# smallflyingpig/speech-to-image-translation-without-text

Measured on AMD Instinct MI355X. Metric: StackGAN-v2 3-stage G+D train-step images/sec at 256px, higher is better.
Workload: dtype f32

## Files before the change

### include/s2i_hip.h

```cpp
#ifndef S2I_HIP_H
#define S2I_HIP_H

#include <stddef.h>
#include <stdint.h>

#ifdef __cplusplus
extern "C" {
#endif

#define S2I_ABI_VERSION 4

#define S2I_CONV_K1      0
#define S2I_CONV_K3S1    1
#define S2I_CONV_K4S2    2
#define S2I_TCONV_K4S2   3

#define S2I_CONV_1D      4

#define S2I_ACT_NONE     0
#define S2I_ACT_GLU      1
#define S2I_ACT_LRELU    2
#define S2I_ACT_TANH     3
#define S2I_ACT_RELU     4

// ... 37 lines not shown
                     void* stream);

int s2i_conv_forward_cls(const s2i_conv_desc* d, const float* x, const float* cvec, const float* w,
                         const float* bias, const float* cls_bias, float* y, float* part, void* ws,
                         size_t ws_bytes, void* stream);

int s2i_conv_forward_in(const s2i_conv_desc* d, const float* x_raw, const float* in_coef, const float* w, float* y,
                        float* part, void* ws, size_t ws_bytes, void* stream);

int s2i_cvec_bias_table(const float* cvec, const float* packed, int B, int Cc, int Ip, int Op, int N,
                        float* table, void* ws , size_t ws_bytes, void* stream);
size_t s2i_border_sums_workspace_bytes(int B, int H, int W, int C);
int s2i_tap_sums(const float* dy, int B, int H, int W, int C, float* tapsum, void* ws, size_t ws_bytes,
                 void* stream);
int s2i_cvec_grads(const float* cvec, const float* packed, const float* tapsum, int B, int Cc, int Ip,
                   int Op, int N, int O, int I_total, float* dc, float* dw_oihw, int accumulate,
                   void* stream);

typedef struct s2i_wgrad_desc {
  int kind;
  int B, H, W;
  int Ca;
  int Cc;
  int N;
  int ldg;
  int swap;
  int fold;
  int O, I, KH, KW;
  int accumulate;
  int i_off;
  int I_total;
  int a_act;
  int a_groups;
} s2i_wgrad_desc;

size_t s2i_wgrad_workspace_bytes(const s2i_wgrad_desc* d);
int s2i_conv_wgrad(const s2i_wgrad_desc* d, const float* a, const float* cvec, const float* g,
                   float* grad_oihw, void* ws, size_t ws_bytes, void* stream);

int s2i_conv_wgrad_in_eligible(const s2i_wgrad_desc* d);
int s2i_conv_wgrad_in(const s2i_wgrad_desc* d, const float* a_raw, const float* a_coef, const float* g,
                      float* grad_oihw, void* ws, size_t ws_bytes, void* stream);


int s2i_conv_split_eligible(const s2i_conv_desc* d);
int s2i_conv_forward_split(const s2i_conv_desc* d, const float* x, const float* cvec,
                           const unsigned short* wsplit, int planes, int np, int kp, const float* bias,
                           const float* cls_bias, float* y, float* part, void* ws, size_t ws_bytes,
                           void* stream);
size_t s2i_wgrad_workspace_bytes_split(const s2i_wgrad_desc* d, int planes);
int s2i_conv_wgrad_split(const s2i_wgrad_desc* d, int planes, const float* a, const float* cvec,
                         const float* g, float* grad_oihw, void* ws, size_t ws_bytes, void* stream);
int s2i_split_packed_weight(const float* packed, int T, int R, int C, int planes, unsigned short* out_rc,
                            unsigned short* out_cr, void* stream);


int    s2i_conv_bf16_eligible(const s2i_conv_desc* d);
size_t s2i_conv_bf16_workspace_bytes(const s2i_conv_desc* d);
int    s2i_conv_bf16_stat_parts(const s2i_conv_desc* d);
size_t s2i_conv_bf16_weight_elems(const s2i_conv_desc* d);
int    s2i_conv_bf16_weight_layout(const s2i_conv_desc* d);
int s2i_pack_conv_weight_bf16(const s2i_conv_desc* d, const float* packed, int R, int C, unsigned short* out,
                              void* stream);
typedef struct s2i_pack16_item {
  const float* P;
  unsigned short* out;
// ... 123 lines not shown
```

### speech_to_image_translation_without_text_amd/_lib.py

```python
import ctypes
import os

import torch

_HERE = os.path.dirname(os.path.abspath(__file__))
LIB_PATH = os.path.join(_HERE, "libs2i_hip.so")

CONV_K1, CONV_K3S1, CONV_K4S2, TCONV_K4S2, CONV_1D = 0, 1, 2, 3, 4
ACT_NONE, ACT_GLU, ACT_LRELU, ACT_TANH, ACT_RELU = 0, 1, 2, 3, 4
PACK_PLAIN, PACK_UPFOLD = 0, 1
DT_F32, DT_BF16 = 0, 1
ABI_VERSION = 4

c_int, c_float, c_void_p, c_size_t, c_ll = (ctypes.c_int, ctypes.c_float, ctypes.c_void_p,
                                            ctypes.c_size_t, ctypes.c_longlong)


class ConvDesc(ctypes.Structure):
    _fields_ = [(n, c_int) for n in ("kind", "B", "H", "W", "Cx", "Cc", "N", "wmode", "flip", "wR",
                                     "ldw", "act", "stats", "ldy", "groups", "nosplit", "kw", "stride", "pad",
                                     "tile_rows", "in_act", "in_groups")]


class WgradDesc(ctypes.Structure):
    _fields_ = [(n, c_int) for n in ("kind", "B", "H", "W", "Ca", "Cc", "N", "ldg", "swap", "fold",
                                     "O", "I", "KH", "KW", "accumulate", "i_off", "I_total", "a_act", "a_groups")]


class PackItem(ctypes.Structure):
    _fields_ = [("w", c_void_p), ("packed", c_void_p)] + [(n, c_int) for n in ("O", "I", "KH", "KW", "Ip", "mode", "gx",
                                                                               "block0")]


class Pack16Item(ctypes.Structure):
    _fields_ = [("P", c_void_p), ("out", c_void_p)] + [(n, c_int) for n in (
        "R", "C", "kind", "flip", "transpose", "T", "nphase", "Nn", "Npad", "Kk", "CK", "gx", "gy", "block0")]


P = c_void_p
_SIGNATURES = {
    "s2i_last_error": (ctypes.c_char_p, []),
    "s2i_version": (c_int, []),
    "s2i_check_device": (c_int, []),
    "s2i_set_tuning": (c_int, [ctypes.c_char_p, c_int]),
    "s2i_get_tuning": (c_int, [ctypes.c_char_p, ctypes.POINTER(c_int)]),
    "s2i_conv_workspace_bytes": (c_size_t, [ctypes.POINTER(ConvDesc)]),
    "s2i_conv_stat_parts": (c_int, [ctypes.POINTER(ConvDesc)]),
    "s2i_conv_forward": (c_int, [ctypes.POINTER(ConvDesc), P, P, P, P, P, P, P, c_size_t, P]),
    "s2i_conv_forward_cls": (c_int, [ctypes.POINTER(ConvDesc), P, P, P, P, P, P, P, P, c_size_t, P]),
    "s2i_conv_forward_in": (c_int, [ctypes.POINTER(ConvDesc), P, P, P, P, P, P, c_size_t, P]),
    "s2i_conv_wgrad_in_eligible": (c_int, [ctypes.POINTER(WgradDesc)]),
    "s2i_conv_wgrad_in": (c_int, [ctypes.POINTER(WgradDesc), P, P, P, P, P, c_size_t, P]),
    "s2i_conv_split_eligible": (c_int, [ctypes.POINTER(ConvDesc)]),
    "s2i_conv_forward_split": (c_int, [ctypes.POINTER(ConvDesc), P, P, P, c_int, c_int, c_int, P, P, P, P, P, c_size_t, P]),
    "s2i_split_packed_weight": (c_int, [P, c_int, c_int, c_int, c_int, P, P, P]),
    "s2i_wgrad_workspace_bytes_split": (c_size_t, [ctypes.POINTER(WgradDesc), c_int]),
    "s2i_conv_wgrad_split": (c_int, [ctypes.POINTER(WgradDesc), c_int, P, P, P, P, P, c_size_t, P]),
    "s2i_conv_bf16_eligible": (c_int, [ctypes.POINTER(ConvDesc)]),
    "s2i_conv_bf16_workspace_bytes": (c_size_t, [ctypes.POINTER(ConvDesc)]),
# ... 153 lines not shown
```

### speech_to_image_translation_without_text_amd/csrc/s2i_igemm.hip

```cpp
#include "s2i_common.h"

namespace {

struct IgemmP {
  const float* __restrict__ x;
  const float* __restrict__ cvec;
  const float* __restrict__ w;
  const float* __restrict__ bias;
  const float* __restrict__ cls_bias;
  float* __restrict__ y;
  float* __restrict__ part;
  float* __restrict__ slab;
  int B, H, W, Cx, Cc, Ca;
  int Ho, Wo, lgWo, lgHoWo;
  int M, N, K, T;
  int kind, flip, act, stats, splitk, cps, nchunks;
  int ldw, wR, ldy, nparts;
  int g_kw, g_s, g_pad;
  int wt;
  int x16, y16;
  unsigned x_bytes, c_bytes, w_bytes;
  long long Mrows;
  const unsigned short* __restrict__ wsp;
  int wsp_np, wsp_kp, wsp_plane;
// ... 1259 lines not shown
      } else {
        *reinterpret_cast<f32x4*>(y + row * ldy + quad * 4) = v;
      }
      s0 += v;
      s1 += v * v;
    }
  }
  sh[0][tid] = s0;
  sh[1][tid] = s1;
  __syncthreads();
  if (rl == 0 && quad < Q) {
    for (int r = 1; r < rpb; ++r) {
      s0 += sh[0][r * cpb + ql];
      s1 += sh[1][r * cpb + ql];
    }
    *reinterpret_cast<f32x4*>(part + ((size_t)0 * nparts + blockIdx.x) * N + quad * 4) = s0;
    *reinterpret_cast<f32x4*>(part + ((size_t)1 * nparts + blockIdx.x) * N + quad * 4) = s1;
  }
}

struct WgradP {
  const float* __restrict__ a;
  const float* __restrict__ cvec;
  const float* __restrict__ g;
  float* __restrict__ slab;
  int B, H, W, Ca, Cc, Cin;
  int Ho, Wo, lgWo, lgHoWo;
  int M, N, ldg, K, T, kind;
  int cps, nchunks;
  int a16, g16;
  unsigned a_bytes, c_bytes, g_bytes;
  const float* __restrict__ a_coef;
  int a_groups, a_ipg;
};

__device__ __forceinline__ void wgrad_block_map(int& tile, int& split) {
  const int tiles = gridDim.x * gridDim.y, nsplit = gridDim.z;
  const int L = blockIdx.x + gridDim.x * (blockIdx.y + gridDim.y * blockIdx.z);
  const int per_group = 8 * tiles;
  const int grp = L / per_group, Ll = L - grp * per_group;
  const int in_group = min(8, nsplit - grp * 8);
  split = grp * 8 + Ll % in_group;
  tile = Ll / in_group;
}

template <int BM, int BN, int WAVES_M, int WAVES_N, bool AACT = false>
__global__ __launch_bounds__(64 * WAVES_M * WAVES_N, (WAVES_M * WAVES_N > 4 ? 4 : 3)) void igemm_wgrad_kernel(WgradP p) {
  constexpr int TM = BM / (WAVES_M * 32), TN = BN / (WAVES_N * 32);
  constexpr int LDA = BM, LDB = BN;
  constexpr int NT = 64 * WAVES_M * WAVES_N;
  constexpr int AROWS = NT * 4 / BM, BROWS = NT * 4 / BN;
  static_assert(AROWS * BM == NT * 4 && BROWS * BN == NT * 4, "a pass must cover whole rows");
  constexpr int APASS = (32 + AROWS - 1) / AROWS, BPASS = (32 + BROWS - 1) / BROWS;
  constexpr bool APRED = (32 % AROWS) != 0, BPRED = (32 % BROWS) != 0;
  __shared__ __attribute__((aligned(16))) float smem[32 * LDA + 32 * LDB];
  float* As = smem;
  float* Bs = smem + 32 * LDA;
  const int tid = threadIdx.x, lane = tid & 63, wave = tid >> 6;
  const int wm = wave / WAVES_N, wn = wave % WAVES_N;
  int tile_, split;
  wgrad_block_map(tile_, split);
  const int k0 = (tile_ % gridDim.x) * BM, n0 = (tile_ / gridDim.x) * BN;
  int s, pad, kw;
  geom(p.kind, s, pad, kw);

  const int acol4 = tid % (BM / 4), arow = tid / (BM / 4);
  const int bcol4 = tid % (BN / 4), brow = tid / (BN / 4);
  const int kcol = k0 + acol4 * 4;
  const bool kvalid = kcol < p.K;
  int c = 0, dy = 0, dx = 0;
  if (kvalid) {
    const int t = kcol / p.Cin;
    c = kcol - t * p.Cin;
    dy = t / kw;
    dx = t - dy * kw;
  }
  const bool from_vec = c < p.Cc;
  const int nb = n0 + bcol4 * 4;
  const bool nvalid = nb < p.N;

  const __amdgpu_buffer_rsrc_t ra_rs = __builtin_amdgcn_make_buffer_rsrc((void*)p.a, 0, p.a_bytes, 0x00020000);
  const __amdgpu_buffer_rsrc_t rc_rs = __builtin_amdgcn_make_buffer_rsrc((void*)p.cvec, 0, p.c_bytes, 0x00020000);
  const __amdgpu_buffer_rsrc_t rg_rs = __builtin_amdgcn_make_buffer_rsrc((void*)p.g, 0, p.g_bytes, 0x00020000);
  const int acolb = (c - p.Cc) * 4;
  const int ccolb = c * 4;
  const int gcolb = nvalid ? nb * 4 : S2I_OOB;
  f32x4 ra[APASS], rb[BPASS];
  f32x4 gs[3], gt[3];
  unsigned apass = 0;
  if constexpr (AACT) {
#pragma unroll
    for (int g = 0; g < 3; ++g) {
      const int gg = g < p.a_groups ? g : 0;
      gs[g] = kvalid ? *reinterpret_cast<const f32x4*>(p.a_coef + ((size_t)gg * 4 + 2) * p.Ca + c) : f32x4{0.f, 0.f, 0.f, 0.f};
      gt[g] = kvalid ? *reinterpret_cast<const f32x4*>(p.a_coef + ((size_t)gg * 4 + 3) * p.Ca + c) : f32x4{0.f, 0.f, 0.f, 0.f};
    }
  }
  auto fetch = [&](int pc) {
    if constexpr (AACT) apass = 0;
#pragma unroll
    for (int q = 0; q < APASS; ++q) {
      const int m = pc * 32 + arow + q * AROWS;
      if (APRED && arow + q * AROWS >= 32) continue;
      const int b = m >> p.lgHoWo;
      const int r = m & ((1 << p.lgHoWo) - 1);
      const int oy = r >> p.lgWo, ox = r & (p.Wo - 1);
// ... 24 lines not shown

  const int c_begin = split * p.cps;
  const int c_end = min(p.nchunks, c_begin + p.cps);
  if (c_begin < c_end) fetch(c_begin);
  for (int pc = c_begin; pc < c_end; ++pc) {
#pragma unroll
    for (int q = 0; q < APASS; ++q)
      if (!APRED || arow + q * AROWS < 32) {
        f32x4 v = ra[q];
        if constexpr (AACT) {
          const unsigned bits = (apass >> (3 * q)) & 7u;
          const unsigned grp = bits & 3u;
          const f32x4 sc = grp == 0 ? gs[0] : (grp == 1 ? gs[1] : gs[2]);
          const f32x4 sh = grp == 0 ? gt[0] : (grp == 1 ? gt[1] : gt[2]);
#pragma unroll
          for (int j = 0; j < 4; ++j) {
            float z = fmaf(v[j], sc[j], sh[j]);
            z = z > 0.f ? z : 0.2f * z;
            v[j] = (bits & 4u) ? z : 0.f;
          }
        }
        *reinterpret_cast<f32x4*>(As + (arow + q * AROWS) * LDA + acol4 * 4) = v;
      }
#pragma unroll
    for (int q = 0; q < BPASS; ++q)
      if (!BPRED || brow + q * BROWS < 32) *reinterpret_cast<f32x4*>(Bs + (brow + q * BROWS) * LDB + bcol4 * 4) = rb[q];
    __syncthreads();
    if (pc + 1 < c_end) fetch(pc + 1);
    mma_chunk<TM, TN, LDA, LDB>(As, Bs, wm * TM * 32, wn * TN * 32, lane, acc);
    __syncthreads();
  }

  const int l31 = lane & 31, lh = lane >> 5;
  float* outp = p.slab + (size_t)split * p.K * p.N;
#pragma unroll
  for (int i = 0; i < TM; ++i)
#pragma unroll
    for (int r = 0; r < 16; ++r) {
      const int krow = k0 + wm * TM * 32 + i * 32 + (r & 3) + 8 * (r >> 2) + 4 * lh;
      if (krow >= p.K) continue;
#pragma unroll
      for (int j = 0; j < TN; ++j) {
        const int n = n0 + wn * TN * 32 + j * 32 + l31;
        if (n < p.N) outp[(size_t)krow * p.N + n] = acc[i][j][r];
      }
    }
}

typedef short s16x4 __attribute__((ext_vector_type(4)));
typedef short s16x8 __attribute__((ext_vector_type(8)));

__device__ __forceinline__ s16x4 lds_tr_read(const unsigned char* ptr) {
  return __builtin_amdgcn_ds_read_tr16_b64_v4i16((s16x4 __attribute__((address_space(3)))*)(ptr));
}

template <int BM, int BN, int WAVES_M, int WAVES_N, int NP>
__global__ __launch_bounds__(256, 3) void igemm_wgrad_split_kernel(WgradP p) {
  constexpr int TM = BM / (WAVES_M * 32), TN = BN / (WAVES_N * 32);
  constexpr int AROWB = BM * 2, BROWB = BN * 2;
  constexpr int APLANE = 32 * AROWB, BPLANE = 32 * BROWB;
  constexpr int AMASK = BM / 8 - 1, BMASK = BN / 8 - 1;
  constexpr int APASS = BM / 32, BPASS = BN / 32;
  constexpr int AROWS = 1024 / BM, BROWS = 1024 / BN;
  __shared__ __attribute__((aligned(16))) unsigned char smem[NP * (APLANE + BPLANE)];
  unsigned char* As = smem;
  unsigned char* Bs = smem + NP * APLANE;
// ... 477 lines not shown
    f32x4 g0[9], g1[9];
    const f32x4 av0 = load_a(m0), av1 = load_a(m1);
    load_g(m0, g0);
    load_g(m1, g1);
    fma9(av0, g0);
    fma9(av1, g1);
  }
  if (grp < ngroups) {
    const int m0 = grp * PPW + pl;
    f32x4 g0[9];
    const f32x4 av0 = load_a(m0);
    load_g(m0, g0);
    fma9(av0, g0);
  }
#pragma unroll
  for (int t = 0; t < 9; ++t)
#pragma unroll
    for (int j = 0; j < 4; ++j) {
      f32x4 v = acc[t][j];
#pragma unroll
      for (int sft = LPP; sft < 64; sft <<= 1)
#pragma unroll
        for (int n = 0; n < 4; ++n) v[n] += __shfl_xor(v[n], sft);
      if (pl == 0) red[wave][(t * LPP + q) * 4 + j] = v;
    }
  __syncthreads();
  float* outp = p.slab + (size_t)blockIdx.x * p.K * 4;
  for (int e = tid; e < 9 * LPP * 4; e += 256) {
    const f32x4 v = red[0][e] + red[1][e] + red[2][e] + red[3][e];
    *reinterpret_cast<f32x4*>(outp + (size_t)e * 4) = v;
  }
}

__global__ __launch_bounds__(256) void slab_sum_tree_kernel(float* __restrict__ slab, int S, int n4) {
  __shared__ f32x4 sh[256];
  const int tid = threadIdx.x;
  const int e = blockIdx.x * 4 + (tid & 3), sl = tid >> 2;
  f32x4 v = {0.f, 0.f, 0.f, 0.f};
  if (e < n4)
    for (int s = sl; s < S; s += 64) v += *reinterpret_cast<const f32x4*>(slab + ((size_t)s * n4 + e) * 4);
  sh[tid] = v;
  __syncthreads();
  for (int h = 32; h >= 1; h >>= 1) {
    if (sl < h) sh[tid] += sh[tid + h * 4];
    __syncthreads();
  }
  if (sl == 0 && e < n4) *reinterpret_cast<f32x4*>(slab + (size_t)e * 4) = sh[tid];
}

__global__ __launch_bounds__(256) void slab_sum_kernel(float* __restrict__ slab, int S, long long n4) {
  for (long long e = (long long)blockIdx.x * blockDim.x + threadIdx.x; e < n4;
       e += (long long)gridDim.x * blockDim.x) {
    f32x4 v = *reinterpret_cast<const f32x4*>(slab + e * 4);
    for (int s = 1; s < S; ++s) v += *reinterpret_cast<const f32x4*>(slab + ((size_t)s * n4 + e) * 4);
    *reinterpret_cast<f32x4*>(slab + e * 4) = v;
  }
}

__global__ __launch_bounds__(256) void wgrad_finish_kernel(const float* __restrict__ slab, int S, int K, int N,
                                                           int Cg, int O, int I, int Tp, int T, int swap, int fold,
                                                           int accumulate, int RT, float* __restrict__ grad,
                                                           int i_off, int I_total) {
  extern __shared__ float tile[];
  const int tid = threadIdx.x;
  const int ncols = swap ? I : O, nrows = swap ? O : I;
  const int c0 = blockIdx.x * 32, r0 = blockIdx.y * RT;
  const size_t sstride = (size_t)K * N;
  const int nload = T * RT * 32;
  for (int e = tid; e < nload; e += 256) {
    const int c_l = e & 31;
    const int r_l = (e >> 5) % RT;
    const int t = (e >> 5) / RT;
    const int c = c0 + c_l, r = r0 + r_l;
    float v = 0.f;
    if (c < ncols && r < nrows) {
      const float* sp = slab + ((size_t)t * Cg + r) * N + c;
      for (int s = 0; s < S; ++s) v += sp[s * sstride];
    }
    tile[(t * RT + r_l) * 33 + c_l] = v;
  }
  __syncthreads();
  const int nout = 32 * RT * Tp;
  for (int w = tid; w < nout; w += 256) {
    const int tapo = w % Tp;
    const int rest = w / Tp;
    int o_l, i_l, r_l, c_l;
    if (swap) { i_l = rest & 31; o_l = rest >> 5; r_l = o_l; c_l = i_l; }
    else { i_l = rest % RT; o_l = rest / RT; r_l = i_l; c_l = o_l; }
// ... 718 lines not shown
}

extern "C" size_t s2i_wgrad_workspace_bytes_dt(const s2i_wgrad_desc* d, int a_dtype, int g_dtype) {
  WgPlan pl;
  if (plan_wgrad(d, &pl, (a_dtype && g_dtype) ? 16 : ((a_dtype || g_dtype) ? 1 : 0))) return 0;
  return (size_t)pl.splitk * pl.K * d->N * sizeof(float);
}

extern "C" int s2i_conv_wgrad_dt(const s2i_wgrad_desc* d, const void* a, int a_dtype, const float* cvec, const void* g,
                                 int g_dtype, float* grad_oihw, void* ws, size_t ws_bytes, void* stream) {
  S2I_REQUIRE((a_dtype == S2I_DT_F32 || a_dtype == S2I_DT_BF16) && (g_dtype == S2I_DT_F32 || g_dtype == S2I_DT_BF16),
              "wgrad: unknown dtype");
  return conv_wgrad_impl(d, 0, (const float*)a, cvec, (const float*)g, grad_oihw, ws, ws_bytes, stream,
                         a_dtype == S2I_DT_BF16, g_dtype == S2I_DT_BF16);
}

extern "C" int s2i_conv_wgrad(const s2i_wgrad_desc* d, const float* a, const float* cvec, const float* g,
                              float* grad_oihw, void* ws, size_t ws_bytes, void* stream) {
  return conv_wgrad_impl(d, 0, a, cvec, g, grad_oihw, ws, ws_bytes, stream);
}

extern "C" size_t s2i_wgrad_workspace_bytes_split(const s2i_wgrad_desc* d, int planes) {
  WgPlan pl;
  if (plan_wgrad(d, &pl, planes)) return 0;
  return (size_t)pl.splitk * pl.K * d->N * sizeof(float);
}

extern "C" int s2i_conv_wgrad_split(const s2i_wgrad_desc* d, int planes, const float* a, const float* cvec,
                                    const float* g, float* grad_oihw, void* ws, size_t ws_bytes, void* stream) {
  S2I_REQUIRE(planes >= 1 && planes <= 3, "wgrad(split): need 1 to 3 bf16 planes");
  return conv_wgrad_impl(d, planes, a, cvec, g, grad_oihw, ws, ws_bytes, stream);
}

template <int BM, int BN, int WM, int WN>
static void launch_wgrad_split(const WgradP& p, dim3 grid, int planes, hipStream_t st) {
  if (planes == 1) hipLaunchKernelGGL((igemm_wgrad_split_kernel<BM, BN, WM, WN, 1>), grid, dim3(256), 0, st, p);
  else if (planes == 2) hipLaunchKernelGGL((igemm_wgrad_split_kernel<BM, BN, WM, WN, 2>), grid, dim3(256), 0, st, p);
  else hipLaunchKernelGGL((igemm_wgrad_split_kernel<BM, BN, WM, WN, 3>), grid, dim3(256), 0, st, p);
}

static int conv_wgrad_impl(const s2i_wgrad_desc* d, int planes, const float* a, const float* cvec, const float* g,
                           float* grad_oihw, void* ws, size_t ws_bytes, void* stream, int a16, int g16, const float* a_coef) {
  WgPlan pl;
  if (plan_wgrad(d, &pl, (a16 && g16) ? 16 : ((planes || a16 || g16) ? 1 : 0))) return 1;
  S2I_REQUIRE(!(planes && (a16 || g16)), "wgrad(split): bf16 tensors go through s2i_conv_wgrad_dt");
  S2I_REQUIRE(!(pl.small_n && g16), "wgrad: the <= 4 channel gradient stream expects an fp32 output gradient");
  S2I_REQUIRE((a || d->Ca == 0) && g && grad_oihw, "wgrad: null operand");
  S2I_REQUIRE(d->Cc == 0 || cvec != nullptr, "wgrad: cvec is null but Cc > 0");
  const size_t need = (size_t)pl.splitk * pl.K * d->N * sizeof(float);
  S2I_REQUIRE(ws && ws_bytes >= need, "wgrad: workspace too small (%zu < %zu)", ws_bytes, need);
  hipStream_t st = (hipStream_t)stream;
  WgradP p;
  p.a = a; p.cvec = cvec; p.g = g; p.slab = (float*)ws;
  p.B = d->B; p.H = d->H; p.W = d->W; p.Ca = d->Ca; p.Cc = d->Cc; p.Cin = pl.Cin;
  p.Ho = pl.Ho; p.Wo = pl.Wo; p.lgWo = s2i_ilog2(pl.Wo); p.lgHoWo = s2i_ilog2(pl.Ho * pl.Wo);
  p.M = pl.M; p.N = d->N; p.ldg = d->ldg; p.K = pl.K; p.T = pl.T; p.kind = d->kind;
  p.cps = pl.cps; p.nchunks = pl.nchunks;
  p.a16 = a16; p.g16 = g16;
  p.a_coef = a_coef; p.a_groups = d->a_groups < 1 ? 1 : d->a_groups; p.a_ipg = d->B / p.a_groups;
  if (a_coef) {
    S2I_REQUIRE(!planes && !a16 && !g16 && wgrad_in_ok(d, pl),
                "wgrad(apply-on-load): fp32 operands, LeakyReLU producer, no broadcast vector, 128 x 128 tile plan (check "
                "s2i_conv_wgrad_in_eligible)");
  }
  {
    const unsigned long long ab = (unsigned long long)d->B * d->H * d->W * d->Ca * (a16 ? 2ull : 4ull);
    const unsigned long long gb = (unsigned long long)pl.M * d->ldg * (g16 ? 2ull : 4ull);
    S2I_REQUIRE(ab < 0x7ff00000ull && gb < 0x7ff00000ull, "wgrad: tensor exceeds the 2 GiB buffer-addressing window");
    p.a_bytes = (unsigned)ab; p.g_bytes = (unsigned)gb;
    p.c_bytes = (unsigned)((unsigned long long)d->B * d->Cc * 4ull);
  }
  dim3 grid(pl.gridK, pl.gridN, pl.splitk);
  if (!a16 && g16 && d->kind == S2I_CONV_K4S2 && d->Ca == 4 && d->Cc == 0 && pl.K == 64 && d->N <= 64 && (d->N % 8) == 0 &&
      (d->ldg % 8) == 0) {
    WgradP q = p;
    q.nchunks = s2i_cdiv(pl.M, 64);
    q.cps = s2i_cdiv(q.nchunks, pl.splitk);
    dim3 g32(1, 1, s2i_cdiv(q.nchunks, q.cps));
    pl.splitk = (int)g32.z;
    pl.gridK = 1; pl.gridN = 1;
    hipLaunchKernelGGL((igemm_wgrad_b16_kernel<64, 64, 2, 2, true>), g32, dim3(256), 0, st, q);
  } else if (a16 && g16 && !pl.small_n && d->Cc == 0 && (pl.Cin % 8) == 0 && (d->N % 8) == 0 && (d->ldg % 8) == 0) {
    WgradP q = p;
    q.nchunks = s2i_cdiv(pl.M, 64);
    q.cps = s2i_cdiv(q.nchunks, pl.splitk);
    dim3 g16grid(pl.gridK, pl.gridN, s2i_cdiv(q.nchunks, q.cps));
    S2I_REQUIRE((int)g16grid.z <= pl.splitk, "wgrad(bf16): split plan mismatch");
    pl.splitk = (int)g16grid.z;
    if (pl.tile == 7) hipLaunchKernelGGL((igemm_wgrad_b16_kernel<256, 256, 4, 4>), g16grid, dim3(1024), 0, st, q);
    else if (pl.tile == 6) hipLaunchKernelGGL((igemm_wgrad_b16_kernel<256, 128, 4, 2>), g16grid, dim3(512), 0, st, q);
    else if (pl.tile == 0) hipLaunchKernelGGL((igemm_wgrad_b16_kernel<128, 128, 2, 2>), g16grid, dim3(256), 0, st, q);
    else if (pl.tile == 1) hipLaunchKernelGGL((igemm_wgrad_b16_kernel<128, 64, 2, 2>), g16grid, dim3(256), 0, st, q);
    else if (pl.tile == 2) hipLaunchKernelGGL((igemm_wgrad_b16_kernel<128, 32, 4, 1>), g16grid, dim3(256), 0, st, q);
    else hipLaunchKernelGGL((igemm_wgrad_b16_kernel<64, 64, 2, 2>), g16grid, dim3(256), 0, st, q);
  } else if (pl.rows3) {
    dim3 g3(d->Ca == 32 ? 1 : 3, pl.gridN, pl.splitk);
    if (d->Ca == 32 && pl.bn3 == 64) hipLaunchKernelGGL((wgrad_k3_rows_kernel<32, 64, 3, 1, 3>), g3, dim3(192), 0, st, p);
    else if (d->Ca == 32) hipLaunchKernelGGL((wgrad_k3_rows_kernel<32, 32, 3, 1, 3>), g3, dim3(192), 0, st, p);
    else if (pl.bn3 == 128) hipLaunchKernelGGL((wgrad_k3_rows_kernel<64, 128, 2, 2, 1>), g3, dim3(256), 0, st, p);
    else if (pl.bn3 == 64) hipLaunchKernelGGL((wgrad_k3_rows_kernel<64, 64, 2, 2, 1>), g3, dim3(256), 0, st, p);
    else hipLaunchKernelGGL((wgrad_k3_rows_kernel<64, 32, 2, 1, 1>), g3, dim3(128), 0, st, p);
  } else if (planes && !pl.small_n) {
    if (pl.tile == 0) launch_wgrad_split<128, 128, 2, 2>(p, grid, planes, st);
    else if (pl.tile == 1) launch_wgrad_split<128, 64, 2, 2>(p, grid, planes, st);
    else if (pl.tile == 2) launch_wgrad_split<128, 32, 4, 1>(p, grid, planes, st);
    else launch_wgrad_split<64, 64, 2, 2>(p, grid, planes, st);
  } else if (pl.small_n) {
    if (d->Ca == 16) hipLaunchKernelGGL(small_n_wgrad_kernel<4>, dim3(pl.splitk), dim3(256), 0, st, p);
    else if (d->Ca == 32) hipLaunchKernelGGL(small_n_wgrad_kernel<8>, dim3(pl.splitk), dim3(256), 0, st, p);
    else hipLaunchKernelGGL(small_n_wgrad_kernel<16>, dim3(pl.splitk), dim3(256), 0, st, p);
  } else if (pl.tile == 9) hipLaunchKernelGGL((igemm_wgrad_kernel<256, 256, 4, 4>), grid, dim3(1024), 0, st, p);
  else if (pl.tile == 8) hipLaunchKernelGGL((igemm_wgrad_kernel<256, 128, 4, 2>), grid, dim3(512), 0, st, p);
  else if (pl.tile == 0 && a_coef) hipLaunchKernelGGL((igemm_wgrad_kernel<128, 128, 2, 2, true>), grid, dim3(256), 0, st, p);
  else if (pl.tile == 0) hipLaunchKernelGGL((igemm_wgrad_kernel<128, 128, 2, 2>), grid, dim3(256), 0, st, p);
  else if (pl.tile == 1) hipLaunchKernelGGL((igemm_wgrad_kernel<128, 64, 2, 2>), grid, dim3(256), 0, st, p);
  else if (pl.tile == 2) hipLaunchKernelGGL((igemm_wgrad_kernel<128, 32, 4, 1>), grid, dim3(256), 0, st, p);
  else if (pl.tile == 3) hipLaunchKernelGGL((igemm_wgrad_kernel<64, 64, 2, 2>), grid, dim3(256), 0, st, p);
  else if (pl.tile == 4) hipLaunchKernelGGL((igemm_wgrad_kernel<96, 64, 3, 1>), grid, dim3(192), 0, st, p);
  else hipLaunchKernelGGL((igemm_wgrad_kernel<96, 32, 3, 1>), grid, dim3(192), 0, st, p);
  S2I_LAUNCH_CHECK("igemm_wgrad");
  {
    const int ncols = d->swap ? d->I : d->O, nrows = d->swap ? d->O : d->I;
    int RT = 8;
    while (RT > 1 && (long long)s2i_cdiv(ncols, 32) * s2i_cdiv(nrows, RT) < 128) RT >>= 1;
    dim3 fgrid(s2i_cdiv(ncols, 32), s2i_cdiv(nrows, RT));
    const size_t shb = (size_t)pl.T * RT * 33 * sizeof(float);
    int S = pl.splitk;
    const long long kn = (long long)pl.K * d->N;
    if (pl.small_n || (S >= 32 && (kn % 4) == 0 && kn / 4 < (1 << 18))) {
      hipLaunchKernelGGL(slab_sum_tree_kernel, dim3(s2i_cdiv(kn / 4, 4)), dim3(256), 0, st, (float*)ws, S, (int)(kn / 4));
      S2I_LAUNCH_CHECK("slab_sum_tree");
      S = 1;
    } else if (S > 2 && (kn % 4) == 0) {
      int sb = s2i_cdiv(kn / 4, 256);
      if (sb > 4096) sb = 4096;
      hipLaunchKernelGGL(slab_sum_kernel, dim3(sb), dim3(256), 0, st, (float*)ws, S, kn / 4);
      S2I_LAUNCH_CHECK("slab_sum");
      S = 1;
    }
    hipLaunchKernelGGL(wgrad_finish_kernel, fgrid, dim3(256), shb, st, (const float*)ws, S, pl.K, d->N,
                       pl.Cin, d->O, d->I, d->KH * d->KW, pl.T, d->swap, d->fold, d->accumulate, RT, grad_oihw,
                       d->i_off, d->I_total > 0 ? d->I_total : d->I);
  }
  S2I_LAUNCH_CHECK("wgrad_finish");
  return 0;
}

extern "C" int s2i_pack_conv_weights_batched(const s2i_pack_item* items_dev, int n, int total_blocks, int max_taps,
                                             void* stream) {
  S2I_REQUIRE(items_dev && n > 0 && total_blocks > 0 && max_taps > 0 && max_taps <= 16, "pack(batched): bad args");
  const size_t shb = (size_t)64 * (8 * max_taps + 1) * sizeof(float);
  hipLaunchKernelGGL(pack_weight_batched_kernel, dim3(total_blocks), dim3(256), shb, (hipStream_t)stream, items_dev, n);
  S2I_LAUNCH_CHECK("pack_weight_batched");
  return 0;
}

extern "C" int s2i_pack_conv_weight(const float* w_oihw, float* packed, int O, int I, int KH, int KW, int Ip,
                                    int mode, void* stream) {
  S2I_REQUIRE(w_oihw && packed, "pack: null pointer");
  S2I_REQUIRE(O > 0 && I > 0 && KH > 0 && KW > 0 && Ip >= I, "pack: bad shape");
  int T = KH * KW;
  if (mode == S2I_PACK_UPFOLD) {
    S2I_REQUIRE(KH == 3 && KW == 3, "pack: UPFOLD needs a 3x3 parameter");
    T = 16;
  } else {
    S2I_REQUIRE(mode == S2I_PACK_PLAIN, "pack: unknown mode %d", mode);
  }
  const int Op = (O + 3) & ~3;
  {
// ... 9 lines not shown
```

### speech_to_image_translation_without_text_amd/ops.py

```python
import ctypes
import os

import torch

from . import _lib
from ._lib import (ACT_GLU, ACT_LRELU, ACT_NONE, CONV_K1, CONV_K3S1, CONV_K4S2, DT_BF16, DT_F32,
                   PACK_PLAIN, PACK_UPFOLD, TCONV_K4S2, ConvDesc, WgradDesc, check, ptr, stream)

BN_EPS = 1e-5
BN_MOMENTUM = 0.1

DIRECT_PARAM_GRAD = False


def _direct(p):
    return (DIRECT_PARAM_GRAD and p is not None and p.requires_grad and p.grad is not None
            and p.grad.is_contiguous())


class param_grad_mode:

    def __init__(self, direct=True):
        self.new = bool(direct)

# ... 371 lines not shown
    y = torch.empty((B, Ho, Wo, N), dtype=torch.float32, device=x.device)
    if EXEC_LOG is not None:
        T = kw1 if conv1d is not None else _TAPS[kind]
        _log_exec("conv k%d %s[%d,%d,%d,%d+%d]->%d" % (kind, "T" if wmode else "", B, H, W, Cx, Cc, N), B * Ho * Wo, N,
                  T * (Cx + Cc), x.numel(), T * (Cx + Cc) * N * (4 if kind == TCONV_K4S2 else 1), y.numel())
    part, nparts = None, 0
    if stats:
        nparts = lib.s2i_conv_stat_parts(ctypes.byref(d))
        if nparts <= 0:
            check(1, "s2i_conv_stat_parts")
        part = torch.empty((2, nparts, N), dtype=torch.float32, device=x.device)
    wsb = lib.s2i_conv_workspace_bytes(ctypes.byref(d))
    ws = _ws.get(wsb, x.device)
    if (MATH_PLANES and in_src is None and w_offset == 0 and packed.dim() == 3
            and getattr(packed, '_s2i_gen', None) is not None and lib.s2i_conv_split_eligible(ctypes.byref(d))):
        transpose = wmode == 0
        np_, kp = (packed.shape[2], packed.shape[1]) if transpose else (packed.shape[1], packed.shape[2])
        if kp % 8 == 0:
            wsp = split_weight(packed, MATH_PLANES, transpose)
            check(lib.s2i_conv_forward_split(ctypes.byref(d), ptr(x), ptr(cvec), ptr(wsp), MATH_PLANES, np_, kp, ptr(bias),
                                             ptr(cls_bias), ptr(y), ptr(part), ptr(ws), ws.numel() * 4, stream()),
                  "s2i_conv_forward_split")
            return y, part, nparts
    wp = ptr(packed) + 4 * int(w_offset)
    if in_src is not None:
        check(lib.s2i_conv_forward_in(ctypes.byref(d), ptr(x), ptr(in_src.coef), wp, ptr(y), ptr(part), ptr(ws),
                                      ws.numel() * 4, stream()), "s2i_conv_forward_in")
        return y, part, nparts
    check(lib.s2i_conv_forward_cls(ctypes.byref(d), ptr(x), ptr(cvec), wp, ptr(bias), ptr(cls_bias), ptr(y), ptr(part),
                                   ptr(ws), ws.numel() * 4, stream()), "s2i_conv_forward")
    return y, part, nparts


def wgrad_raw(kind, a, cvec, g, grad_shape, *, swap=0, fold=0, out=None, accumulate=False, i_off=0, I_total=0, a_src=None):
    lib = _lib_ready()
    B, H, W, Ca = a.shape
    Cc = 0 if cvec is None else cvec.shape[1]
    N = g.shape[-1]
    if len(grad_shape) == 2:
        O, I, KH, KW = grad_shape[0], grad_shape[1], 1, 1
    else:
        O, I, KH, KW = grad_shape
    d = WgradDesc(kind, B, H, W, Ca, Cc, N, N, swap, fold, O, I, KH, KW, 1 if accumulate else 0, i_off, I_total,
                  a_src.act if a_src is not None else 0, a_src.groups if a_src is not None else 0)
    if EXEC_LOG is not None:
        Ho, Wo = _geom(kind, H, W)
        _log_exec("wgrad k%d a[%d,%d,%d,%d+%d] g%d" % (kind, B, H, W, Ca, Cc, N), B * Ho * Wo, N, _TAPS[kind] * (Ca + Cc),
                  a.numel(), g.numel(), _TAPS[kind] * (Ca + Cc) * N)
    if out is None:
        full = grad_shape if not I_total else (O, I_total, KH, KW)
        out = torch.empty(full, dtype=torch.float32, device=a.device)
    if a_src is not None:
        wsb = lib.s2i_wgrad_workspace_bytes(ctypes.byref(d))
        if wsb == 0:
            check(1, "s2i_wgrad_workspace_bytes")
        ws = _ws.get(wsb, a.device)
        check(lib.s2i_conv_wgrad_in(ctypes.byref(d), ptr(a), ptr(a_src.coef), ptr(g), ptr(out), ptr(ws), ws.numel() * 4,
                                    stream()), "s2i_conv_wgrad_in")
        return out
    if MATH_PLANES:
        wsb = lib.s2i_wgrad_workspace_bytes_split(ctypes.byref(d), MATH_PLANES)
        if wsb == 0:
            check(1, "s2i_wgrad_workspace_bytes_split")
        ws = _ws.get(wsb, a.device)
        check(lib.s2i_conv_wgrad_split(ctypes.byref(d), MATH_PLANES, ptr(a), ptr(cvec), ptr(g), ptr(out), ptr(ws),
                                       ws.numel() * 4, stream()), "s2i_conv_wgrad_split")
        return out
    wsb = lib.s2i_wgrad_workspace_bytes(ctypes.byref(d))
    if wsb == 0:
        check(1, "s2i_wgrad_workspace_bytes")
    ws = _ws.get(wsb, a.device)
    check(lib.s2i_conv_wgrad(ctypes.byref(d), ptr(a), ptr(cvec), ptr(g), ptr(out), ptr(ws), ws.numel() * 4,
                             stream()), "s2i_conv_wgrad")
    return out


def _rows_view(t):
# ... 617 lines not shown
```

Measured before the change: 748.4.

## Write conv wgrad results directly in OIHW layout, fusing the relayout and tap fold

```diff
diff --git a/include/s2i_hip.h b/include/s2i_hip.h
--- a/include/s2i_hip.h
+++ b/include/s2i_hip.h
@@ -93,6 +93,7 @@
   int I_total;
   int a_act;
   int a_groups;
+  int slab_finish;
 } s2i_wgrad_desc;
 
 size_t s2i_wgrad_workspace_bytes(const s2i_wgrad_desc* d);
diff --git a/speech_to_image_translation_without_text_amd/_lib.py b/speech_to_image_translation_without_text_amd/_lib.py
--- a/speech_to_image_translation_without_text_amd/_lib.py
+++ b/speech_to_image_translation_without_text_amd/_lib.py
@@ -24,7 +24,8 @@
 
 class WgradDesc(ctypes.Structure):
     _fields_ = [(n, c_int) for n in ("kind", "B", "H", "W", "Ca", "Cc", "N", "ldg", "swap", "fold",
-                                     "O", "I", "KH", "KW", "accumulate", "i_off", "I_total", "a_act", "a_groups")]
+                                     "O", "I", "KH", "KW", "accumulate", "i_off", "I_total", "a_act", "a_groups",
+                                     "slab_finish")]
 
 
 class PackItem(ctypes.Structure):
diff --git a/speech_to_image_translation_without_text_amd/csrc/s2i_igemm.hip b/speech_to_image_translation_without_text_amd/csrc/s2i_igemm.hip
--- a/speech_to_image_translation_without_text_amd/csrc/s2i_igemm.hip
+++ b/speech_to_image_translation_without_text_amd/csrc/s2i_igemm.hip
@@ -1315,6 +1315,9 @@
   unsigned a_bytes, c_bytes, g_bytes;
   const float* __restrict__ a_coef;
   int a_groups, a_ipg;
+  float* __restrict__ grad;
+  int I_total, i_off, accumulate;
+  int fold;
 };
 
 __device__ __forceinline__ void wgrad_block_map(int& tile, int& split) {
@@ -1327,7 +1330,7 @@
   tile = Ll / in_group;
 }
 
-template <int BM, int BN, int WAVES_M, int WAVES_N, bool AACT = false>
+template <int BM, int BN, int WAVES_M, int WAVES_N, bool AACT = false, bool OIHW = false>
 __global__ __launch_bounds__(64 * WAVES_M * WAVES_N, (WAVES_M * WAVES_N > 4 ? 4 : 3)) void igemm_wgrad_kernel(WgradP p) {
   constexpr int TM = BM / (WAVES_M * 32), TN = BN / (WAVES_N * 32);
   constexpr int LDA = BM, LDB = BN;
@@ -1352,9 +1355,17 @@
   const int kcol = k0 + acol4 * 4;
   const bool kvalid = kcol < p.K;
   int c = 0, dy = 0, dx = 0;
+  constexpr int OG = BM / 16;
   if (kvalid) {
-    const int t = kcol / p.Cin;
-    c = kcol - t * p.Cin;
+    int t;
+    if constexpr (OIHW) {
+      const int rl = acol4 * 4;
+      t = rl / OG;
+      c = k0 / 16 + rl % OG;
+    } else {
+      t = kcol / p.Cin;
+      c = kcol - t * p.Cin;
+    }
     dy = t / kw;
     dx = t - dy * kw;
   }
@@ -1445,6 +1456,58 @@
   }
 
   const int l31 = lane & 31, lh = lane >> 5;
+  if constexpr (OIHW) {
+    constexpr int LDT = BM + 4;
+    const bool one = gridDim.z == 1;
+    float* dst = one ? p.grad + (size_t)p.i_off * 16 : p.slab + (size_t)split * p.K * p.N;
+    const size_t ostride = one ? (size_t)p.I_total * 16 : (size_t)p.Cin * 16;
+    dst += k0;
+#pragma unroll
+    for (int cw = 0; cw < WAVES_N; ++cw)
+#pragma unroll
+      for (int j = 0; j < TN; ++j) {
+        __syncthreads();
+        if (wn == cw) {
+#pragma unroll
+          for (int i = 0; i < TM; ++i)
+#pragma unroll
+            for (int r = 0; r < 16; ++r) {
+              const int row = wm * TM * 32 + i * 32 + (r & 3) + 8 * (r >> 2) + 4 * lh;
+              smem[l31 * LDT + (row % OG) * 16 + row / OG] = acc[i][j][r];
+            }
+        }
+        __syncthreads();
+        for (int e = (one && p.fold) ? NT * 32 * BM : tid; e < 32 * (BM / 4); e += NT) {
+          const int col = e / (BM / 4), q = e - col * (BM / 4);
+          const int n = n0 + cw * TN * 32 + j * 32 + col;
+          if (n >= p.N) continue;
+          f32x4 v = *reinterpret_cast<const f32x4*>(smem + col * LDT + q * 4);
+          f32x4* gp = reinterpret_cast<f32x4*>(dst + (size_t)n * ostride + q * 4);
+          if (one) {
+            v = f32x4{0.f, 0.f, 0.f, 0.f} + v;
+            if (p.accumulate) v = *gp + v;
+          }
+          *gp = v;
+        }
+        if (one && p.fold) {
+          for (int e = tid; e < OG * 32 * 9; e += NT) {
+            const int ol = e / 288, rest = e - ol * 288, col = rest / 9, tap = rest - col * 9;
+            const int n = n0 + cw * TN * 32 + j * 32 + col;
+            if (n >= p.N) continue;
+            const float* x = smem + col * LDT + ol * 16;
+            const int ky = tap / 3, kx = tap - ky * 3;
+            float v = 0.f;
+#pragma unroll
+            for (int ay = 0; ay < 2; ++ay)
+#pragma unroll
+              for (int ax = 0; ax < 2; ++ax) v += 0.f + x[((2 - ky) + ay) * 4 + (2 - kx) + ax];
+            float* gp = p.grad + ((size_t)(k0 / 16 + ol) * p.I_total + p.i_off + n) * 9 + tap;
+            *gp = p.accumulate ? *gp + v : v;
+          }
+        }
+      }
+    return;
+  }
   float* outp = p.slab + (size_t)split * p.K * p.N;
 #pragma unroll
   for (int i = 0; i < TM; ++i)
@@ -1988,7 +2051,44 @@
   }
 }
 
-__global__ __launch_bounds__(256) void slab_sum_tree_kernel(float* __restrict__ slab, int S, int n4) {
+struct SlabToGrad {
+  float* grad;
+  int run, gstride, goff, accumulate;
+  int fold;
+};
+
+__device__ __forceinline__ void slab_fold_store(const SlabToGrad& og, long long grp, const f32x4 (&x)[4]) {
+  const long long i = grp / og.run, o = grp - i * og.run;
+  float* gp = og.grad + ((size_t)o * og.gstride + og.goff + i) * 9;
+#pragma unroll
+  for (int tap = 0; tap < 9; ++tap) {
+    const int ky = tap / 3, kx = tap - ky * 3;
+    float v = 0.f;
+#pragma unroll
+    for (int ay = 0; ay < 2; ++ay)
+#pragma unroll
+      for (int ax = 0; ax < 2; ++ax) {
+        const int t = ((2 - ky) + ay) * 4 + (2 - kx) + ax;
+        v += 0.f + x[t >> 2][t & 3];
+      }
+    gp[tap] = og.accumulate ? gp[tap] + v : v;
+  }
+}
+
+__device__ __forceinline__ void slab_sum_store(float* __restrict__ slab, const SlabToGrad& og, long long e4, f32x4 v) {
+  if (!og.grad) {
+    *reinterpret_cast<f32x4*>(slab + e4 * 4) = v;
+    return;
+  }
+  const long long e = e4 * 4;
+  const long long o = e / og.run;
+  f32x4* gp = reinterpret_cast<f32x4*>(og.grad + o * og.gstride + og.goff + (e - o * og.run));
+  v = f32x4{0.f, 0.f, 0.f, 0.f} + v;
+  if (og.accumulate) v = *gp + v;
+  *gp = v;
+}
+
+__global__ __launch_bounds__(256) void slab_sum_tree_kernel(float* __restrict__ slab, int S, int n4, SlabToGrad og) {
   __shared__ f32x4 sh[256];
   const int tid = threadIdx.x;
   const int e = blockIdx.x * 4 + (tid & 3), sl = tid >> 2;
@@ -2001,15 +2101,34 @@
     if (sl < h) sh[tid] += sh[tid + h * 4];
     __syncthreads();
   }
-  if (sl == 0 && e < n4) *reinterpret_cast<f32x4*>(slab + (size_t)e * 4) = sh[tid];
-}
-
-__global__ __launch_bounds__(256) void slab_sum_kernel(float* __restrict__ slab, int S, long long n4) {
+  if (og.fold) {
+    if (tid == 0 && e < n4) {
+      const f32x4 x[4] = {sh[0], sh[1], sh[2], sh[3]};
+      slab_fold_store(og, blockIdx.x, x);
+    }
+    return;
+  }
+  if (sl == 0 && e < n4) slab_sum_store(slab, og, e, sh[tid]);
+}
+
+__global__ __launch_bounds__(256) void slab_sum_kernel(float* __restrict__ slab, int S, long long n4, SlabToGrad og) {
+  if (og.fold) {
+    for (long long g = (long long)blockIdx.x * blockDim.x + threadIdx.x; g < n4 / 4; g += (long long)gridDim.x * blockDim.x) {
+      f32x4 x[4];
+#pragma unroll
+      for (int q = 0; q < 4; ++q) {
+        x[q] = *reinterpret_cast<const f32x4*>(slab + (g * 4 + q) * 4);
+        for (int s = 1; s < S; ++s) x[q] += *reinterpret_cast<const f32x4*>(slab + ((size_t)s * n4 + g * 4 + q) * 4);
+      }
+      slab_fold_store(og, g, x);
+    }
+    return;
+  }
   for (long long e = (long long)blockIdx.x * blockDim.x + threadIdx.x; e < n4;
        e += (long long)gridDim.x * blockDim.x) {
     f32x4 v = *reinterpret_cast<const f32x4*>(slab + e * 4);
     for (int s = 1; s < S; ++s) v += *reinterpret_cast<const f32x4*>(slab + ((size_t)s * n4 + e) * 4);
-    *reinterpret_cast<f32x4*>(slab + e * 4) = v;
+    slab_sum_store(slab, og, e, v);
   }
 }
 
@@ -2794,6 +2913,19 @@
   return conv_wgrad_impl(d, planes, a, cvec, g, grad_oihw, ws, ws_bytes, stream);
 }
 
+static bool wgrad_oihw_ok(const s2i_wgrad_desc* d, const WgPlan& pl, int planes, int a16, int g16) {
+  if (d->slab_finish || planes || a16 || g16 || pl.rows3 || pl.small_n) return false;
+  if (d->kind != S2I_CONV_K4S2 || d->Cc != 0) return false;
+  if (d->swap && d->fold) {
+    if (d->KH != 3 || d->KW != 3 || pl.Cin != d->O || d->N != d->I) return false;
+  } else if (d->swap || d->fold || d->KH != 4 || d->KW != 4 || pl.Cin != d->I || d->N != d->O) {
+    return false;
+  }
+  const int BM = pl.tile == 3 ? 64 : ((pl.tile == 8 || pl.tile == 9) ? 256 : 128);
+  if (!(pl.tile <= 3 || pl.tile == 8 || pl.tile == 9)) return false;
+  return (pl.K % BM) == 0;
+}
+
 template <int BM, int BN, int WM, int WN>
 static void launch_wgrad_split(const WgradP& p, dim3 grid, int planes, hipStream_t st) {
   if (planes == 1) hipLaunchKernelGGL((igemm_wgrad_split_kernel<BM, BN, WM, WN, 1>), grid, dim3(256), 0, st, p);
@@ -2820,6 +2952,9 @@
   p.cps = pl.cps; p.nchunks = pl.nchunks;
   p.a16 = a16; p.g16 = g16;
   p.a_coef = a_coef; p.a_groups = d->a_groups < 1 ? 1 : d->a_groups; p.a_ipg = d->B / p.a_groups;
+  p.grad = grad_oihw; p.I_total = d->I_total > 0 ? d->I_total : d->I; p.i_off = d->i_off; p.accumulate = d->accumulate;
+  p.fold = d->fold;
+  const bool oihw = wgrad_oihw_ok(d, pl, planes, a16, g16);
   if (a_coef) {
     S2I_REQUIRE(!planes && !a16 && !g16 && wgrad_in_ok(d, pl),
                 "wgrad(apply-on-load): fp32 operands, LeakyReLU producer, no broadcast vector, 128 x 128 tile plan (check "
@@ -2871,6 +3006,15 @@
     if (d->Ca == 16) hipLaunchKernelGGL(small_n_wgrad_kernel<4>, dim3(pl.splitk), dim3(256), 0, st, p);
     else if (d->Ca == 32) hipLaunchKernelGGL(small_n_wgrad_kernel<8>, dim3(pl.splitk), dim3(256), 0, st, p);
     else hipLaunchKernelGGL(small_n_wgrad_kernel<16>, dim3(pl.splitk), dim3(256), 0, st, p);
+  } else if (oihw) {
+    if (pl.tile == 9) hipLaunchKernelGGL((igemm_wgrad_kernel<256, 256, 4, 4, false, true>), grid, dim3(1024), 0, st, p);
+    else if (pl.tile == 8) hipLaunchKernelGGL((igemm_wgrad_kernel<256, 128, 4, 2, false, true>), grid, dim3(512), 0, st, p);
+    else if (pl.tile == 0 && a_coef)
+      hipLaunchKernelGGL((igemm_wgrad_kernel<128, 128, 2, 2, true, true>), grid, dim3(256), 0, st, p);
+    else if (pl.tile == 0) hipLaunchKernelGGL((igemm_wgrad_kernel<128, 128, 2, 2, false, true>), grid, dim3(256), 0, st, p);
+    else if (pl.tile == 1) hipLaunchKernelGGL((igemm_wgrad_kernel<128, 64, 2, 2, false, true>), grid, dim3(256), 0, st, p);
+    else if (pl.tile == 2) hipLaunchKernelGGL((igemm_wgrad_kernel<128, 32, 4, 1, false, true>), grid, dim3(256), 0, st, p);
+    else hipLaunchKernelGGL((igemm_wgrad_kernel<64, 64, 2, 2, false, true>), grid, dim3(256), 0, st, p);
   } else if (pl.tile == 9) hipLaunchKernelGGL((igemm_wgrad_kernel<256, 256, 4, 4>), grid, dim3(1024), 0, st, p);
   else if (pl.tile == 8) hipLaunchKernelGGL((igemm_wgrad_kernel<256, 128, 4, 2>), grid, dim3(512), 0, st, p);
   else if (pl.tile == 0 && a_coef) hipLaunchKernelGGL((igemm_wgrad_kernel<128, 128, 2, 2, true>), grid, dim3(256), 0, st, p);
@@ -2881,7 +3025,24 @@
   else if (pl.tile == 4) hipLaunchKernelGGL((igemm_wgrad_kernel<96, 64, 3, 1>), grid, dim3(192), 0, st, p);
   else hipLaunchKernelGGL((igemm_wgrad_kernel<96, 32, 3, 1>), grid, dim3(192), 0, st, p);
   S2I_LAUNCH_CHECK("igemm_wgrad");
+  if (oihw) {
+    const int S = pl.splitk;
+    const long long kn = (long long)pl.K * d->N;
+    const SlabToGrad og = d->fold ? SlabToGrad{grad_oihw, pl.Cin, p.I_total, d->i_off, d->accumulate, 1}
+                                  : SlabToGrad{grad_oihw, pl.K, p.I_total * 16, d->i_off * 16, d->accumulate, 0};
+    if (S >= 32 && kn / 4 < (1 << 18)) {
+      hipLaunchKernelGGL(slab_sum_tree_kernel, dim3(s2i_cdiv(kn / 4, 4)), dim3(256), 0, st, (float*)ws, S, (int)(kn / 4), og);
+      S2I_LAUNCH_CHECK("slab_sum_tree");
+    } else if (S > 1) {
+      int sb = s2i_cdiv(d->fold ? kn / 16 : kn / 4, 256);
+      if (sb > 4096) sb = 4096;
+      hipLaunchKernelGGL(slab_sum_kernel, dim3(sb), dim3(256), 0, st, (float*)ws, S, kn / 4, og);
+      S2I_LAUNCH_CHECK("slab_sum");
+    }
+    return 0;
+  }
   {
+    const SlabToGrad to_slab{nullptr, 1, 0, 0, 0, 0};
     const int ncols = d->swap ? d->I : d->O, nrows = d->swap ? d->O : d->I;
     int RT = 8;
     while (RT > 1 && (long long)s2i_cdiv(ncols, 32) * s2i_cdiv(nrows, RT) < 128) RT >>= 1;
@@ -2890,13 +3051,13 @@
     int S = pl.splitk;
     const long long kn = (long long)pl.K * d->N;
     if (pl.small_n || (S >= 32 && (kn % 4) == 0 && kn / 4 < (1 << 18))) {
-      hipLaunchKernelGGL(slab_sum_tree_kernel, dim3(s2i_cdiv(kn / 4, 4)), dim3(256), 0, st, (float*)ws, S, (int)(kn / 4));
+      hipLaunchKernelGGL(slab_sum_tree_kernel, dim3(s2i_cdiv(kn / 4, 4)), dim3(256), 0, st, (float*)ws, S, (int)(kn / 4), to_slab);
       S2I_LAUNCH_CHECK("slab_sum_tree");
       S = 1;
     } else if (S > 2 && (kn % 4) == 0) {
       int sb = s2i_cdiv(kn / 4, 256);
       if (sb > 4096) sb = 4096;
-      hipLaunchKernelGGL(slab_sum_kernel, dim3(sb), dim3(256), 0, st, (float*)ws, S, kn / 4);
+      hipLaunchKernelGGL(slab_sum_kernel, dim3(sb), dim3(256), 0, st, (float*)ws, S, kn / 4, to_slab);
       S2I_LAUNCH_CHECK("slab_sum");
       S = 1;
     }
diff --git a/speech_to_image_translation_without_text_amd/ops.py b/speech_to_image_translation_without_text_amd/ops.py
--- a/speech_to_image_translation_without_text_amd/ops.py
+++ b/speech_to_image_translation_without_text_amd/ops.py
@@ -427,7 +427,8 @@
     return y, part, nparts
 
 
-def wgrad_raw(kind, a, cvec, g, grad_shape, *, swap=0, fold=0, out=None, accumulate=False, i_off=0, I_total=0, a_src=None):
+def wgrad_raw(kind, a, cvec, g, grad_shape, *, swap=0, fold=0, out=None, accumulate=False, i_off=0, I_total=0, a_src=None,
+              slab_finish=0):
     lib = _lib_ready()
     B, H, W, Ca = a.shape
     Cc = 0 if cvec is None else cvec.shape[1]
@@ -437,7 +438,7 @@
     else:
         O, I, KH, KW = grad_shape
     d = WgradDesc(kind, B, H, W, Ca, Cc, N, N, swap, fold, O, I, KH, KW, 1 if accumulate else 0, i_off, I_total,
-                  a_src.act if a_src is not None else 0, a_src.groups if a_src is not None else 0)
+                  a_src.act if a_src is not None else 0, a_src.groups if a_src is not None else 0, slab_finish)
     if EXEC_LOG is not None:
         Ho, Wo = _geom(kind, H, W)
         _log_exec("wgrad k%d a[%d,%d,%d,%d+%d] g%d" % (kind, B, H, W, Ca, Cc, N), B * Ho * Wo, N, _TAPS[kind] * (Ca + Cc),
```

Result: no change. 749.9, median of 6 (+0.2%).
